# iris-ua/iris_lama

Measured on AMD Instinct MI355X. Metric: particle-scans/sec, higher is better.
Workload: dtype f64; 1 GPU; PFSlam2D 30 particles, 1080-beam synthetic corridor log (SURVEY.md 8(d)), res 0.05 m, patch 32, l2_max 0.5, GN+Cauchy(0.15), seed 42; particles=30, beams=1080, parallelism=particle-shard x1

## Files before the change

iris_lama_amd/csrc/lama_hip.hip:

```cpp
#include "../../include/lama_hip.h"

#include <hip/hip_runtime.h>

#include <algorithm>
#include <cmath>
#include <cstdio>
#include <cstdlib>
#include <cstring>
#include <map>
#include <memory>
#include <mutex>
#include <string>
#include <vector>

#include "lama_kernels.h"
#include "lama_pgo.h"
#include "lama_map_build.h"
#include "../host/pgo_pattern.hpp"

using namespace lama_dev;

namespace {

template <class T>
// ... 676 lines not shown
        size_t free_b = 0, total_b = 0;
        if (hipMemGetInfo(&free_b, &total_b) == hipSuccess && 2 * P * nWW * 2 + (1ull << 28) > free_b)
            return fail(c, LAMA_HIP_E_WINDOW, "not enough device memory to re-tile the window directories (" + std::to_string(2 * P * nWW * 2 >> 20) + " MB for a " + std::to_string(newW) + "-patch window)");
    }
    DevBuf<int16_t> nd[2];
    for (int k = 0; k < 2; ++k) {
        hipError_t e = nd[k].alloc(P * nWW);
        if (e == hipSuccess && newW != c->W) e = hipMemsetAsync(nd[k], 0xFF, P * nWW * 2, c->stream);
        if (e != hipSuccess) return hip_fail(c, e, "window directories");
    }
    const dim3 grid((unsigned)P, (unsigned)((std::max(WW, nWW) + 255) / 256));
    int16_t* const to_dm = nd[0]; int16_t* const to_occ = nd[1];
    hipLaunchKernelGGL(k_shift_window, grid, dim3(256), 0, c->stream, c->ms.dm_dir, to_dm, c->W, newW, dx, dy, WW, nWW, c->d_err);
    hipLaunchKernelGGL(k_shift_window, grid, dim3(256), 0, c->stream, c->ms.occ_dir, to_occ, c->W, newW, dx, dy, WW, nWW, c->d_err);
    {
        hipError_t e = hipGetLastError();
        if (e == hipSuccess) e = hipStreamSynchronize(c->stream);
        if (e != hipSuccess) return hip_fail(c, e, "k_shift_window");
    }
    c->ms.dm_dir.swap(nd[0]); c->ms.occ_dir.swap(nd[1]);
    if (newW != c->W) {
        c->W = newW; c->WC = newW * 32; c->cfg.window_patches = newW;
        c->ctr.window_growths += 1;
    }
    c->wx0 = (uint32_t)(nox * 32); c->wy0 = (uint32_t)(noy * 32);
    c->ctr.window_shifts += 1;
    c->ctr.window_patches = c->W;
    return LAMA_HIP_OK;
}

int32_t ensure_window(lama_hip_ctx* c, int64_t x0, int64_t x1, int64_t y0, int64_t y1)
{
    if (!c->mb_valid) { c->mbx0 = x0; c->mbx1 = x1; c->mby0 = y0; c->mby1 = y1; c->mb_valid = true; }
    else { c->mbx0 = std::min(c->mbx0, x0); c->mbx1 = std::max(c->mbx1, x1); c->mby0 = std::min(c->mby0, y0); c->mby1 = std::max(c->mby1, y1); }
    const int64_t ox = c->wx0 >> 5, oy = c->wy0 >> 5, W = c->W;
    if (c->debug_window) std::fprintf(stderr, "ensure_window: box x [%ld, %ld] y [%ld, %ld] mapped x [%ld, %ld] y [%ld, %ld] window x [%ld, %ld) y [%ld, %ld)\n", (long)x0, (long)x1, (long)y0, (long)y1, (long)c->mbx0, (long)c->mbx1, (long)c->mby0, (long)c->mby1, (long)ox, (long)(ox + W), (long)oy, (long)(oy + W));
    if (c->mbx0 >= ox && c->mbx1 < ox + W && c->mby0 >= oy && c->mby1 < oy + W) return LAMA_HIP_OK;
    const int64_t span = std::max(c->mbx1 - c->mbx0 + 1, c->mby1 - c->mby0 + 1);
    int64_t newW = W;
    if (span > W) newW = std::min<int64_t>(LAMA_HIP_MAX_WINDOW, std::max<int64_t>((span + 8 + 7) / 8 * 8, (W + W / 2 + 7) / 8 * 8));
    int64_t hx0 = c->mbx0, hx1 = c->mbx1, hy0 = c->mby0, hy1 = c->mby1;
    if (span > newW) { hx0 = x0; hx1 = x1; hy0 = y0; hy1 = y1; if (x1 - x0 + 1 > newW || y1 - y0 + 1 > newW) return LAMA_HIP_OK; }
    auto place = [&](int64_t o, int64_t lo, int64_t hi) {
        const int64_t a = hi - newW + 1, b = lo;
        int64_t no = std::min(std::max(o, a), b);
        if (no > o) no = std::min(no + 4, b); else if (no < o) no = std::max(no - 4, a);
        return no;
    };
    const int64_t nox = c->initialised ? place(ox, hx0, hx1) : (hx0 + hx1 + 1) / 2 - newW / 2;
    const int64_t noy = c->initialised ? place(oy, hy0, hy1) : (hy0 + hy1 + 1) / 2 - newW / 2;
    return regrid_window(c, (uint32_t)newW, nox, noy);
}

int32_t start_without_first_scan(lama_hip_ctx* c)
{
    if (c->initialised) return LAMA_HIP_OK;
    for (uint32_t p = 0; p < c->P; ++p) { c->h_poses[4 * p] = 1.0; c->h_poses[4 * p + 1] = 0.0; c->h_poses[4 * p + 2] = 0.0; c->h_poses[4 * p + 3] = 0.0; }
    HIPCHK(c, hipMemcpyAsync(c->d_poses, c->h_poses.data(), sizeof(double) * 4 * c->P, hipMemcpyHostToDevice, c->stream));
    c->initialised = true;
    return LAMA_HIP_OK;
}

int32_t fit_window(lama_hip_ctx* c, const Affine& mtf, uint32_t first, uint32_t count)
{
    double far = c->scan_reach;
    if (c->cfg.ray_rule == 0 && c->cfg.truncated_range > 0.0) far = std::min(far, c->cfg.truncated_range);
    const uint32_t guard_r = ((uint32_t)std::ceil(std::sqrt((double)c->max_sqdist)) + 1u + 31u) / 32u;
    const double reach = far + std::sqrt(mtf.t[0] * mtf.t[0] + mtf.t[1] * mtf.t[1]) + (double)(guard_r + 1u) * 32.0 * c->cfg.resolution;
    double xlo = 1e300, xhi = -1e300, ylo = 1e300, yhi = -1e300;
    for (uint32_t p = first; p < first + count; ++p) {
        const double x = c->h_poses[4 * p + 2], y = c->h_poses[4 * p + 3];
        xlo = std::min(xlo, x - reach); xhi = std::max(xhi, x + reach);
        ylo = std::min(ylo, y - reach); yhi = std::max(yhi, y + reach);
    }
    auto patch = [&](double w) { return (int64_t)std::floor((c->scale * w + c->off) / 32.0); };
    return ensure_window(c, patch(xlo), patch(xhi), patch(ylo), patch(yhi));
}

static unsigned xcd_grid(const lama_hip_ctx* c, uint32_t first, uint32_t count)
{
    return (first == 0 && count == c->P) ? (count + 7u) / 8u * 8u : count;
}

int32_t launch_allocation_phase(lama_hip_ctx* c, const DevParams& prm, uint32_t n, uint32_t first, uint32_t count, int alloc_only)
{
    const size_t need = (size_t)c->P * n;
    if (need > c->d_rrec.n) {
        c->d_rrec.reset(); c->d_rbbox.reset(); c->d_rchunk.reset();
        hipError_t e = c->d_rrec.alloc(need);
        if (e == hipSuccess) e = c->d_rbbox.alloc(need);
        if (e == hipSuccess) e = c->d_rchunk.alloc((size_t)c->P * ((n + 63) / 64));
        if (e != hipSuccess) { c->d_rrec.reset(); return hip_fail(c, e, "ray buffers"); }
    }
    hipLaunchKernelGGL(k_ray_hits, dim3(xcd_grid(c, first, count), (n + 255) / 256), dim3(256), 0, c->stream, prm, c->d_pts, (int)n, c->d_tfs, (int)first,
                       c->d_rrec, c->d_rbbox, alloc_only, c->d_rchunk);
    const int rw_seg = count <= 64 ? 4 : 1;
    hipLaunchKernelGGL(k_ray_alloc_walk, dim3(xcd_grid(c, first, count), (n * rw_seg + 255) / 256), dim3(256), 0, c->stream, prm, (const lama_dev::RayRec*)c->d_rrec, (int)n, (int)first, rw_seg);
    double far = c->scan_reach;
    if (c->cfg.truncated_range > 0.0) far = std::min(far, c->cfg.truncated_range);
    const int reach_cells = (int)std::ceil(far * c->scale) + 2;
    hipLaunchKernelGGL(k_occ_reverse_dir, dim3(count), dim3(256), 0, c->stream, prm, (int)first, (const double*)c->d_tfs, reach_cells,
                       c->unguarded_retry ? 1 : 0);
    return LAMA_HIP_OK;
}

static uint32_t route_places(const lama_hip_ctx* c, uint32_t count)
{
    const uint32_t slots = c->num_cus * 12u;
    if (c->route_forced || count >= slots) return c->route_cap;
    return std::min<uint32_t>(c->route_cap, std::max<uint32_t>(8u, (slots - count) / 7u));
}

int32_t run_update_maps(lama_hip_ctx* c, uint32_t n, const Affine& mtf, uint32_t first, uint32_t count)
{
    {
        const int32_t rcw = fit_window(c, mtf, first, count);
        if (rcw) return rcw;
    }
    c->last_mtf = mtf; c->last_first = first; c->last_count = count;
    if (c->recover_depth == 0) { c->saved_visit_bound = c->visit_bound; c->saved_ctr = c->ctr; }
    PinVec<double>& tfs = c->h_tfs;
    tfs.resize((size_t)c->P * 12);
    for (uint32_t p = 0; p < c->P; ++p) host_scan_tf(&c->h_poses[4 * p], mtf, &tfs[12 * (size_t)p]);
    HIPCHK(c, hipMemcpyAsync(c->d_tfs, tfs.data(), sizeof(double) * tfs.size(), hipMemcpyHostToDevice, c->stream));
    DevParams prm = make_params(c);
    bool early_lane = false;
    {
        Timer t(c, &c->ctr.ms_raycast, &c->ctr.launches_raycast);
        (void)hipMemsetAsync(c->d_slow_n, 0, 32 + sizeof(uint64_t) * 4 * c->P, c->stream);
        bool sequential = c->cfg.sequential_raycast == 1 || c->cfg.occupancy_policy == 1 ||
                          c->cfg.ray_rule == 1;
        if (!sequential && (n > 4096u || (uint64_t)n + 4096u > c->cfg.active_capacity)) sequential = true;
        if (!sequential && (uint64_t)c->visit_bound + n >= 65536u) {
            uint32_t m = 0;
            if (c->initialised) {
                (void)hipMemsetAsync(c->d_scalar, 0, sizeof(uint32_t), c->stream);
                hipLaunchKernelGGL(k_occ_max_visited, dim3(c->P), dim3(256), 0, c->stream, prm, c->d_scalar);
                HIPCHK(c, hipMemcpyAsync(&m, c->d_scalar, sizeof(uint32_t), hipMemcpyDeviceToHost, c->stream));
                HIPCHK(c, hipStreamSynchronize(c->stream));
            }
            c->visit_bound = m;
            if ((uint64_t)m + n >= 65536u) { sequential = true; c->ctr.wrap_guard_scans += 1; }
        }
        c->visit_bound = (uint32_t)std::min<uint64_t>((uint64_t)c->visit_bound + n, 65535u);
        if (sequential) c->ctr.sequential_raycast_scans += 1; else c->ctr.parallel_raycast_scans += 1;
        c->last_guarded = c->cfg.ray_rule == 0;
        if (!c->last_guarded) {
            const double side = 32.0 * c->cfg.resolution;
            const double rp = c->scan_reach / side + 2.5;
            const uint32_t bound = (uint32_t)std::min(32767.0, std::ceil(3.1416 * rp * rp));
            std::vector<CapRequest> reqs;
            for (uint32_t p = first; p < first + count; ++p) {
                const HostPart& pr = c->h_part[p];
                const uint32_t nd = std::min<uint32_t>(MAX_PATCHES, round_up32((uint32_t)c->h_counts[2 * p] + bound)), no = std::min<uint32_t>(MAX_PATCHES, round_up32((uint32_t)c->h_counts[2 * p + 1] + bound));
                if (nd > pr.dm_cap || no > pr.occ_cap) reqs.push_back(CapRequest{p, std::max(nd, pr.dm_cap), std::max(no, pr.occ_cap)});
            }
            if (!reqs.empty()) {
                const int32_t rg = set_capacities(c, reqs);
                if (rg) return rg;
                prm = make_params(c);
            }
        }
        if (sequential) {
            if (c->last_guarded) { const int32_t ra = launch_allocation_phase(c, prm, n, first, count, 1); if (ra) return ra; }
            hipLaunchKernelGGL(k_raycast, dim3(count), dim3(UM_BLOCK), 0, c->stream, prm, c->d_pts, (int)n, c->d_tfs, (int)first);
        } else {
            const bool two_waves_e = c->cfg.brushfire_waves == 2 || (c->cfg.brushfire_waves == 0 && count <= BF_TW_MAX_PARTICLES);
            early_lane = c->early_on && two_waves_e && c->cfg.brushfire_mode == 0 && first == 0 && count == c->P &&
                         count >= std::max<uint32_t>(c->route_min_count, c->early_min_count) && c->route_cap > 0;
            uint32_t host_n = 0;
            if (early_lane && c->ll_valid) {
                const uint32_t places = route_places(c, count);
                double mean = 0; for (uint32_t p = 0; p < c->P; ++p) mean += c->h_ll[p]; mean /= c->P;
                const double lim = 2.5 * std::min(mean, 0.0) - 5.0;
                std::vector<std::pair<double, uint32_t>> cand;
                for (uint32_t p = 0; p < c->P; ++p) if (c->h_ll[p] < lim) cand.emplace_back(c->h_ll[p], p);
                if (cand.size() > places) { std::partial_sort(cand.begin(), cand.begin() + places, cand.end()); cand.resize(places); }
                c->h_hlist.resize(256);
                for (auto& e : cand) c->h_hlist[host_n++] = e.second;
                if (host_n) HIPCHK(c, hipMemcpyAsync(c->d_hlist, c->h_hlist.data(), sizeof(uint32_t) * host_n, hipMemcpyHostToDevice, c->stream));
            }
            const bool prev_ok = c->early_ok && c->early_candidates > 0;
            early_lane = early_lane && (host_n > 0 || prev_ok);
            if (early_lane)
                hipLaunchKernelGGL(k_early_list, dim3(1), dim3(256), 0, c->stream, prev_ok ? (const uint8_t*)c->d_heavy : (const uint8_t*)nullptr,
                                   (const uint32_t*)c->d_hlist, host_n, c->d_early, c->d_elist, c->d_slow_n + 4, (int)c->P, route_places(c, count));
            { const int32_t ra = launch_allocation_phase(c, prm, n, first, count, 0); if (ra) return ra; }
#ifdef LAMA_WAVE_SIM
            const unsigned gy = 4u;
#else
            const unsigned gy = count <= 64 ? 128u : (count >= 1024 ? 8u : 32u);
#endif
            if (early_lane) {
                DevParams pe = prm;
                pe.elist = c->d_elist; pe.elist_n = c->d_slow_n + 4; pe.lane = 1;
                const unsigned eg = route_places(c, count);
                hipLaunchKernelGGL(k_ray_patches, dim3(eg, 128u), dim3(256), 0, c->stream, pe, (const lama_dev::RayRec*)c->d_rrec,
                                   (const uint64_t*)c->d_rbbox, (const lama_dev::RayChunk*)c->d_rchunk, (int)n, 0);
                hipLaunchKernelGGL((k_ray_replay<RP_SORT_SMALL, RP_SORT_SMALL, false, RP_BLOCK_LARGE>), dim3(eg), dim3(RP_BLOCK_LARGE), 0, c->stream, pe, 0);
                hipLaunchKernelGGL((k_ray_replay<8192, 8192, true, RP_BLOCK_LARGE>), dim3(eg), dim3(RP_BLOCK_LARGE), 0, c->stream, pe, 0);
                HIPCHK(c, hipEventRecord(c->ev_alloc, c->stream));
                HIPCHK(c, hipStreamWaitEvent(c->stream3, c->ev_alloc, 0));
                hipLaunchKernelGGL(k_mark_early, dim3(1), dim3(64), 0, c->stream3, pe);
                HIPCHK(c, hipEventRecord(c->ev_go, c->stream3));
                hipLaunchKernelGGL((k_brushfire<LQ_BIG, RQ_BIG, true, true>), dim3(eg), dim3(2 * UM_BLOCK), c->big_stage_pad, c->stream3, pe, 0, 2);
                HIPCHK(c, hipEventRecord(c->ev_early, c->stream3));
                HIPCHK(c, hipStreamWaitEvent(c->stream, c->ev_go, 0));
                prm.early = c->d_early;
            }
            hipLaunchKernelGGL(k_ray_patches, dim3(xcd_grid(c, first, count), gy), dim3(256), 0, c->stream, prm, (const lama_dev::RayRec*)c->d_rrec,
                               (const uint64_t*)c->d_rbbox, (const lama_dev::RayChunk*)c->d_rchunk, (int)n, (int)first);
            const unsigned resume_grid = std::min<unsigned>(count, 256u);
            if (count <= 512) {
                hipLaunchKernelGGL((k_ray_replay<RP_SORT_SMALL, RP_SORT_SMALL, false, RP_BLOCK_LARGE>), dim3(count), dim3(RP_BLOCK_LARGE), 0, c->stream, prm, (int)first);
                hipLaunchKernelGGL((k_ray_replay<8192, 8192, true, RP_BLOCK_LARGE>), dim3(resume_grid), dim3(RP_BLOCK_LARGE), 0, c->stream, prm, (int)first);
            } else {
                hipLaunchKernelGGL((k_ray_replay<RP_SORT_SMALL, RP_SORT_SMALL, false, RP_BLOCK_SMALL>), dim3(count), dim3(RP_BLOCK_SMALL), 0, c->stream, prm, (int)first);
                hipLaunchKernelGGL((k_ray_replay<8192, 8192, true, RP_BLOCK_SMALL>), dim3(resume_grid), dim3(RP_BLOCK_SMALL), 0, c->stream, prm, (int)first);
            }
        }
        t.stop();
    }
    HIPCHK(c, hipGetLastError());
    {
        Timer t(c, &c->ctr.ms_brushfire, &c->ctr.launches_brushfire);
        if (c->cfg.brushfire_mode == 1)
            hipLaunchKernelGGL(k_brushfire_canon, dim3(count), dim3(CN_BLOCK), 0, c->stream, prm, (int)first);
        const bool two_waves = c->cfg.brushfire_waves == 2 || (c->cfg.brushfire_waves == 0 && count <= BF_TW_MAX_PARTICLES);
        c->ctr.brushfire_mode = c->cfg.brushfire_mode;
        c->ctr.brushfire_waves = two_waves ? 2u : 1u;
        const unsigned resume_grid = std::min<unsigned>(count, 256u);
        const bool route = two_waves && count >= c->route_min_count && c->route_cap > 0;
        if (two_waves) {
            if (route) {
                prm.heavy = c->d_heavy;
                hipLaunchKernelGGL(k_bf_route, dim3(1), dim3(256), 0, c->stream, prm, (int)first, (int)count, c->route_min_events, c->route_percent, route_places(c, count));
                HIPCHK(c, hipEventRecord(c->ev_route, c->stream));
                hipLaunchKernelGGL((k_brushfire<LQ_BIG, RQ_BIG, true, true>), dim3(route_places(c, count)), dim3(2 * UM_BLOCK), 0, c->stream, prm, (int)first, 1);
                HIPCHK(c, hipStreamWaitEvent(c->stream2, c->ev_route, 0));
                hipLaunchKernelGGL((k_brushfire<LQ_SMALL, RQ_SMALL, false, true>), dim3(count), dim3(2 * UM_BLOCK), 0, c->stream2, prm, (int)first, 0);
                HIPCHK(c, hipEventRecord(c->ev_heavy, c->stream2));
                HIPCHK(c, hipStreamWaitEvent(c->stream, c->ev_heavy, 0));
            } else {
                hipLaunchKernelGGL((k_brushfire<LQ_SMALL, RQ_SMALL, false, true>), dim3(count), dim3(2 * UM_BLOCK), 0, c->stream, prm, (int)first, 0);
            }
            hipLaunchKernelGGL((k_brushfire<LQ_BIG, RQ_BIG, true, true>), dim3(resume_grid), dim3(2 * UM_BLOCK), 0, c->stream, prm, (int)first, 0);
        } else {
            hipLaunchKernelGGL((k_brushfire<LQ_SMALL, RQ_SMALL, false, false>), dim3(count), dim3(UM_BLOCK), 0, c->stream, prm, (int)first, 0);
            hipLaunchKernelGGL((k_brushfire<LQ_BIG, RQ_BIG, true, false>), dim3(resume_grid), dim3(UM_BLOCK), 0, c->stream, prm, (int)first, 0);
        }
        if (early_lane) HIPCHK(c, hipStreamWaitEvent(c->stream, c->ev_early, 0));
        hipLaunchKernelGGL(k_brushfire_slow, dim3(count), dim3(UM_BLOCK), 0, c->stream, prm, (int)first);
        c->early_ok = route && first == 0 && count == c->P;
        t.stop();
    }
    HIPCHK(c, hipGetLastError());
    return LAMA_HIP_OK;
}


int32_t permute_particles(lama_hip_ctx* c, const int32_t* idx)
{
    const uint32_t P = c->P;
    std::vector<uint8_t> taken(P, 0);
    std::vector<HostPart> np(P);
    std::vector<int32_t> nc(2 * (size_t)P);
    std::vector<double> npose(4 * (size_t)P);
    std::vector<uint32_t> clones;
    for (uint32_t i = 0; i < P; ++i) {
        const uint32_t j = (uint32_t)idx[i];
// ... 1435 lines not shown
```

iris_lama_amd/csrc/lama_raycast_par.h:

```cpp
#pragma once
#include "lama_dev.h"

namespace lama_dev {


constexpr int RP_BLOCK_SMALL = 256, RP_BLOCK_LARGE = 1024;
#ifdef LAMA_TEST_SMALL_QUEUES
constexpr int RP_SORT_SMALL = 512;
#else
constexpr int RP_SORT_SMALL = 2048;
#endif

__device__ inline int dir_alloc_one(int16_t* dir, uint32_t pidx, int32_t* count, int cap, int errbit, int32_t* err)
{
    uint32_t* w = reinterpret_cast<uint32_t*>(dir) + (pidx >> 1);
    const int sh = (int)(pidx & 1u) * 16;
    for (uint32_t spins = 0;; ++spins) {
        const uint32_t v = __hip_atomic_load(w, __ATOMIC_RELAXED, __HIP_MEMORY_SCOPE_AGENT);
        const int s = (int)(int16_t)((v >> sh) & 0xFFFFu);
        if (s >= 0) return s;
        if (s == -3) return -1;
        if (spins > (1u << 22)) { atomicOr(err, errbit); return -1; }
        if (s == -1) {
            const uint32_t locked = (v & ~(0xFFFFu << sh)) | (0xFFFEu << sh);
// ... 28 lines not shown
        const int leader = __ffsll((long long)m) - 1;
        const uint32_t klo = (uint32_t)__builtin_amdgcn_readlane((int)(uint32_t)key, leader);
        const uint32_t khi = (uint32_t)__builtin_amdgcn_readlane((int)(uint32_t)(key >> 32), leader);
        int r = 0;
        if (lane == leader) r = dir_alloc_one(dir, pidx, count, cap, errbit, err);
        r = __builtin_amdgcn_readlane(r, leader);
        if (pending && (uint32_t)key == klo && (uint32_t)(key >> 32) == khi) { res = r; pending = false; }
    }
    return res;
}

struct BeamGeom {
    uint32_t mhx, mhy, msx, msy;
    uint32_t a0, a1, nn;
    int s0, s1;
    bool mark_hit;
    int steps;
    uint64_t magic;
};

__device__ inline BeamGeom beam_geometry(const DevParams& prm, const double* T, double px, double py, double pz)
{
    double hx = ((T[0] * px + T[1] * py) + T[2] * pz) + T[9];
    double hy = ((T[3] * px + T[4] * py) + T[5] * pz) + T[10];
    double hz = ((T[6] * px + T[7] * py) + T[8] * pz) + T[11];
    double sx = T[9], sy = T[10], sz = T[11];
    double abx = 0, aby = 0, abz = 0, ray_length = 1.0;
    BeamGeom g;
    g.mark_hit = true;
    if (prm.trunc_range > 0.0) {
        abx = hx - sx; aby = hy - sy; abz = hz - sz;
        ray_length = sqrt((abx * abx + aby * aby) + abz * abz);
        if (prm.trunc_range < ray_length) {
            hx = sx + abx / ray_length * prm.trunc_range;
            hy = sy + aby / ray_length * prm.trunc_range;
            hz = sz + abz / ray_length * prm.trunc_range;
            g.mark_hit = false;
        }
    }
    if (g.mark_hit && prm.trunc_ray > 0.0) {
        if (prm.trunc_range == 0.0) {
            abx = hx - sx; aby = hy - sy; abz = hz - sz;
            ray_length = sqrt((abx * abx + aby * aby) + abz * abz);
        }
        if (prm.trunc_ray < ray_length) {
            sx = hx - abx / ray_length * prm.trunc_ray;
            sy = hy - aby / ray_length * prm.trunc_ray;
            sz = hz - abz / ray_length * prm.trunc_ray;
        }
    }
    g.mhx = w2m(prm, hx); g.mhy = w2m(prm, hy);
    g.msx = w2m(prm, sx); g.msy = w2m(prm, sy);
    const uint32_t mhz = w2m(prm, hz), msz = w2m(prm, sz);
    const int64_t d0 = (int64_t)g.mhx - (int64_t)g.msx, d1 = (int64_t)g.mhy - (int64_t)g.msy, d2 = (int64_t)mhz - (int64_t)msz;
    const int64_t a0 = d0 < 0 ? -d0 : d0, a1 = d1 < 0 ? -d1 : d1, a2 = d2 < 0 ? -d2 : d2;
    const int64_t nn = a0 > a1 ? (a0 > a2 ? a0 : a2) : (a1 > a2 ? a1 : a2);
    g.s0 = d0 < 0 ? -1 : 1; g.s1 = d1 < 0 ? -1 : 1;
    g.a0 = (uint32_t)a0; g.a1 = (uint32_t)a1; g.nn = (uint32_t)(nn > 0xFFFFFFFFll ? 0xFFFFFFFFll : nn);
    g.steps = nn > 0 ? (int)g.nn - 1 : 0;
    if (nn >= 8192) g.steps = -1;
    g.magic = (1ull << 42) / (uint64_t)(2 * (nn > 0 && nn < 8192 ? nn : 1)) + 1ull;
    return g;
}

constexpr int ACT_SEQ_BITS = 26, ACT_XY_BITS = 15;
__device__ inline uint64_t act_key(uint32_t rx, uint32_t ry, uint32_t beam, uint32_t t)
{
    return ((uint64_t)((ry << ACT_XY_BITS) | rx) << ACT_SEQ_BITS) | (uint64_t)((beam << 13) | t);
}

__device__ inline void act_append(const DevParams& prm, int p, uint64_t key)
{
    const uint32_t k = atomicAdd(prm.act_count + p, 1u);
    if (k < prm.act_cap) prm.act[(size_t)p * prm.act_cap + k] = key;
    else atomicOr(prm.err, ERR_QUEUE);
}

struct RayRec;
struct RayChunk;
constexpr uint64_t RAY_BBOX_EMPTY = 0x0000FFFF0000FFFFull;
__device__ inline uint64_t ray_hits_record(const DevParams& prm, const BeamGeom& g, int p, int i, int n, RayRec* rec_out, uint64_t* bbox_out);
__device__ inline void ray_chunk_record(const DevParams& prm, const BeamGeom& g, uint64_t bb, int lane, RayChunk* chunks, size_t index);

__global__ __launch_bounds__(256) void k_ray_hits(DevParams prm, const double* __restrict__ pts, int n,
                                                   const double* __restrict__ tfs, int first_particle,
                                                   RayRec* __restrict__ rec_out = nullptr, uint64_t* __restrict__ bbox_out = nullptr, int alloc_only = 0,
                                                   RayChunk* __restrict__ chunk_out = nullptr)
{
    const int p = first_particle + blockIdx.x;
    if (p >= (int)prm.P) return;
    const int i = blockIdx.y * 256 + threadIdx.x;
    const int lane = threadIdx.x & 63;
    const bool live = i < n;
    const int ic = live ? i : n - 1;
    double T[12];
    uload_f64_w<12>(tfs + 12 * (size_t)p, T);
    const BeamGeom g = beam_geometry(prm, T, pts[3 * ic], pts[3 * ic + 1], pts[3 * ic + 2]);
    uint64_t bb = RAY_BBOX_EMPTY;
    if (rec_out && live) bb = ray_hits_record(prm, g, p, i, n, rec_out, bbox_out);
    if (chunk_out && (i & ~63) < n) ray_chunk_record(prm, g, bb, lane, chunk_out, (size_t)p * ((n + 63) / 64) + (i >> 6));
    if (live && g.steps < 0) atomicOr(prm.err, ERR_WINDOW);
    if (!alloc_only) {
        uint32_t st = (live && g.steps > 0) ? (uint32_t)g.steps : 0u;
        for (int off = 32; off > 0; off >>= 1) st += (uint32_t)__shfl_xor((int)st, off, 64);
        if (lane == 0 && st) atomicAdd((unsigned long long*)(prm.stats + 4 * p + 2), (unsigned long long)st);
    }
    bool hit = live && g.steps >= 0 && g.mark_hit;
    const uint32_t rx = g.mhx - prm.wx0, ry = g.mhy - prm.wy0;
    if (hit && (rx >= prm.WC || ry >= prm.WC)) { atomicOr(prm.err, ERR_WINDOW); hit = false; }
    const uint32_t pidx = (ry >> 5) * prm.W + (rx >> 5), ci = (rx & 31u) | ((ry & 31u) << 5);
    int slot = -1;
    const PV pv = pview(prm, p);
    if (hit) slot = dir_get_or_alloc(pv.occ_dir, pidx, prm.counts + 2 * p + 1, (int)pv.occ_cap, ERR_OCC_CAP, prm.err);
    hit = hit && slot >= 0 && !alloc_only;
    if (hit) atomicOr((unsigned long long*)(pv.occ_hit + (size_t)slot * 16 + (ci >> 6)), 1ull << (ci & 63));
    const unsigned long long hm = __ballot(hit);
    if (hm) {
        uint32_t base = 0;
        if (lane == (__ffsll((long long)hm) - 1)) base = atomicAdd(prm.act_count + p, (uint32_t)__popcll(hm));
        base = (uint32_t)__shfl((int)base, __ffsll((long long)hm) - 1, 64);
        if (hit) {
            const uint32_t k = base + (uint32_t)__popcll(hm & ((1ull << lane) - 1ull));
            if (k < prm.act_cap) prm.act[(size_t)p * prm.act_cap + k] = act_key(rx, ry, (uint32_t)i, 0u);
            else atomicOr(prm.err, ERR_QUEUE);
        }
    }
}

template <int RP_BLOCK>
__device__ inline void bitonic_sort(uint64_t* a, uint32_t m)
{
    for (uint32_t k = 2; k <= m; k <<= 1) {
        for (uint32_t j = k >> 1; j > 0; j >>= 1) {
            for (uint32_t i = threadIdx.x; i < m; i += RP_BLOCK) {
                const uint32_t ixj = i ^ j;
                if (ixj > i) {
                    const uint64_t x = a[i], y = a[ixj];
                    const bool up = (i & k) == 0;
                    if ((x > y) == up) { a[i] = y; a[ixj] = x; }
                }
            }
            __syncthreads();
        }
    }
}

template <int RP_BLOCK, int E>
__device__ inline void bitonic_sort_regs(uint64_t* a)
{
    constexpr uint32_t M = (uint32_t)RP_BLOCK * E;
    const uint32_t base = threadIdx.x * (uint32_t)E;
    uint64_t x[E];
#pragma unroll
    for (int r = 0; r < E; ++r) x[r] = a[base + r];
    for (uint32_t k = 2; k <= M; k <<= 1) {
        uint32_t j = k >> 1;
        for (; j >= 64u * E; j >>= 1) {
            __syncthreads();
#pragma unroll
            for (int r = 0; r < E; ++r) a[base + r] = x[r];
            __syncthreads();
            const uint32_t pb = base ^ j;
            const bool keep_min = ((base & j) == 0) == ((base & k) == 0);
#pragma unroll
            for (int r = 0; r < E; ++r) {
                const uint64_t y = a[pb + r];
                x[r] = ((y < x[r]) == keep_min) ? y : x[r];
            }
        }
        for (; j >= (uint32_t)E; j >>= 1) {
            const int lj = (int)(j / (uint32_t)E);
            const bool keep_min = ((base & j) == 0) == ((base & k) == 0);
#pragma unroll
            for (int r = 0; r < E; ++r) {
                const uint64_t y = __shfl_xor(x[r], lj, 64);
                x[r] = ((y < x[r]) == keep_min) ? y : x[r];
            }
        }
#pragma unroll
        for (int jr = E / 2; jr > 0; jr >>= 1) {
            if ((uint32_t)jr >= k) continue;
#pragma unroll
            for (int r = 0; r < E; ++r) {
                if (r & jr) continue;
                const bool up = ((base + (uint32_t)r) & k) == 0;
                const uint64_t lo = x[r], hi = x[r | jr];
                const bool sw = (lo > hi) == up;
                x[r] = sw ? hi : lo; x[r | jr] = sw ? lo : hi;
            }
        }
    }
    __syncthreads();
#pragma unroll
    for (int r = 0; r < E; ++r) a[base + r] = x[r];
    __syncthreads();
}

template <int RP_BLOCK>
__device__ inline void sort_keys(uint64_t* a, uint32_t m)
{
    if (m < (uint32_t)RP_BLOCK) { if (m > 1) bitonic_sort<RP_BLOCK>(a, m); }
    else if (m == (uint32_t)RP_BLOCK) bitonic_sort_regs<RP_BLOCK, 1>(a);
    else if (m == 2u * RP_BLOCK) bitonic_sort_regs<RP_BLOCK, 2>(a);
    else if (m == 4u * RP_BLOCK) bitonic_sort_regs<RP_BLOCK, 4>(a);
    else if (m == 8u * RP_BLOCK) bitonic_sort_regs<RP_BLOCK, 8>(a);
    else bitonic_sort<RP_BLOCK>(a, m);
}

template <int SORT_CAP, int EV_CAP>
// ... 150 lines not shown
```

iris_lama_amd/csrc/lama_raycast_patch.h:

```cpp
#pragma once
#include "lama_raycast_par.h"

namespace lama_dev {

struct RayRec {
    uint32_t msx, msy;
    uint32_t a01;
    uint32_t nnf;
    uint64_t magic;
};
struct RayChunk {
    int32_t cwx, cwy;
    int32_t ccwx, ccwy;
    uint64_t bbox;
    uint32_t sxy;
    uint32_t cone;
};

__device__ inline RayRec ray_rec(const BeamGeom& g)
{
    RayRec r;
    r.msx = g.msx; r.msy = g.msy;
    r.a01 = (g.a0 & 0xFFFFu) | ((g.a1 & 0xFFFFu) << 16);
    r.nnf = (g.nn & 0xFFFFu) | (g.s0 < 0 ? 1u << 16 : 0u) | (g.s1 < 0 ? 1u << 17 : 0u) | (g.steps > 0 ? 1u << 18 : 0u);
    r.magic = g.magic;
    return r;
}
__device__ __forceinline__ void ray_cell(const RayRec& r, uint32_t wx0, uint32_t wy0, uint32_t t, uint32_t& rx, uint32_t& ry)
{
    const uint32_t a0 = r.a01 & 0xFFFFu, a1 = r.a01 >> 16, nn = r.nnf & 0xFFFFu;
    const uint32_t st0 = (uint32_t)(((uint64_t)(2u * t * a0 + nn) * r.magic) >> 42);
    const uint32_t st1 = (uint32_t)(((uint64_t)(2u * t * a1 + nn) * r.magic) >> 42);
    const uint32_t cx = (r.nnf & (1u << 16)) ? r.msx - st0 : r.msx + st0;
    const uint32_t cy = (r.nnf & (1u << 17)) ? r.msy - st1 : r.msy + st1;
    rx = cx - wx0; ry = cy - wy0;
}

__device__ __forceinline__ bool ray_axis_range(int m, bool neg, uint32_t a, uint32_t nn, int lo, uint32_t steps, uint32_t& t_lo, uint32_t& t_hi)
{
    int ka = neg ? m - (lo + 31) : lo - m, kb = neg ? m - lo : lo + 31 - m;
    if (ka < 0) ka = 0;
    if (kb > (int)a) kb = (int)a;
    if (ka > kb) return false;
    t_lo = 1u; t_hi = steps;
    if (a == 0u) return true;
    const uint32_t d = 2u * a;
    if (ka > 0) t_lo = (2u * nn * (uint32_t)ka - nn + d - 1u) / d;
    if (kb < (int)a) t_hi = (2u * nn * (uint32_t)(kb + 1) - nn + d - 1u) / d - 1u;
    if (t_lo < 1u) t_lo = 1u;
    if (t_hi > steps) t_hi = steps;
    return t_lo <= t_hi;
}

__device__ inline uint64_t ray_hits_record(const DevParams& prm, const BeamGeom& g, int p, int i, int n, RayRec* rec_out, uint64_t* bbox_out)
{
    RayRec r = ray_rec(g);
    uint64_t bb = RAY_BBOX_EMPTY;
    bool ok = g.steps > 0;
    if (ok) {
        const int64_t xa = (int64_t)g.msx - (int64_t)prm.wx0, ya = (int64_t)g.msy - (int64_t)prm.wy0;
        const int64_t xb = xa + (int64_t)g.s0 * (int64_t)g.a0, yb = ya + (int64_t)g.s1 * (int64_t)g.a1;
        const int64_t x0 = xa < xb ? xa : xb, x1 = xa < xb ? xb : xa, y0 = ya < yb ? ya : yb, y1 = ya < yb ? yb : ya;
        if (x0 < 0 || y0 < 0 || x1 >= (int64_t)prm.WC || y1 >= (int64_t)prm.WC) { atomicOr(prm.err, ERR_WINDOW); ok = false; }
        else bb = (uint64_t)x0 | ((uint64_t)x1 << 16) | ((uint64_t)y0 << 32) | ((uint64_t)y1 << 48);
    }
    if (!ok) r.nnf &= ~(1u << 18);
    rec_out[(size_t)p * n + i] = r;
    bbox_out[(size_t)p * n + i] = bb;
    return bb;
}

__device__ inline void ray_chunk_record(const DevParams& prm, const BeamGeom& g, uint64_t bb, int lane, RayChunk* chunks, size_t index)
{
    const bool val = bb != RAY_BBOX_EMPTY;
    const unsigned long long vm = __ballot(val);
    uint32_t x0 = (uint32_t)(bb & 0xFFFFu), x1 = (uint32_t)((bb >> 16) & 0xFFFFu), y0 = (uint32_t)((bb >> 32) & 0xFFFFu), y1 = (uint32_t)(bb >> 48);
    for (int off = 32; off > 0; off >>= 1) {
        const uint32_t ox0 = (uint32_t)__shfl_xor((int)x0, off, 64), ox1 = (uint32_t)__shfl_xor((int)x1, off, 64);
        const uint32_t oy0 = (uint32_t)__shfl_xor((int)y0, off, 64), oy1 = (uint32_t)__shfl_xor((int)y1, off, 64);
        x0 = ox0 < x0 ? ox0 : x0; x1 = ox1 > x1 ? ox1 : x1; y0 = oy0 < y0 ? oy0 : y0; y1 = oy1 > y1 ? oy1 : y1;
    }
    const int lf = vm ? __ffsll((long long)vm) - 1 : 0, ll = vm ? 63 - __clzll((long long)vm) : 0;
    const int dx = g.s0 < 0 ? -(int)g.a0 : (int)g.a0, dy = g.s1 < 0 ? -(int)g.a1 : (int)g.a1;
    const int sx = (int)(g.msx - prm.wx0), sy = (int)(g.msy - prm.wy0);
    const int fx = __shfl(dx, lf, 64), fy = __shfl(dy, lf, 64), lx = __shfl(dx, ll, 64), ly = __shfl(dy, ll, 64);
    const int fsx = __shfl(sx, lf, 64), fsy = __shfl(sy, lf, 64);
    const int c_f = fx * dy - fy * dx, c_l = dx * ly - dy * lx;
    const bool front = fx * dx + fy * dy > 0 && lx * dx + ly * dy > 0 && sx == fsx && sy == fsy;
    const bool all_ccw = __ballot(val && !(front && c_f >= 0 && c_l >= 0)) == 0ull;
    const bool all_cw = __ballot(val && !(front && c_f <= 0 && c_l <= 0)) == 0ull;
    if (lane == 0) {
        RayChunk c;
        c.bbox = vm ? ((uint64_t)x0 | ((uint64_t)x1 << 16) | ((uint64_t)y0 << 32) | ((uint64_t)y1 << 48)) : RAY_BBOX_EMPTY;
        c.sxy = ((uint32_t)fsx & 0xFFFFu) | ((uint32_t)fsy << 16);
        c.cone = (vm && (all_ccw || all_cw)) ? 1u : 0u;
        c.cwx = all_ccw ? fx : lx; c.cwy = all_ccw ? fy : ly;
        c.ccwx = all_ccw ? lx : fx; c.ccwy = all_ccw ? ly : fy;
        chunks[index] = c;
    }
}

__global__ __launch_bounds__(256) void k_ray_alloc_walk(DevParams prm, const RayRec* __restrict__ recs, int n, int first_particle, int RW_SEG)
{
    const int p = first_particle + blockIdx.x;
    const int g = blockIdx.y * 256 + threadIdx.x;
    const int i = g / RW_SEG, seg = g % RW_SEG;
    if (i >= n || p >= (int)prm.P) return;
    const RayRec r = recs[(size_t)p * n + i];
    if (!(r.nnf & (1u << 18))) return;
    const uint32_t steps = (r.nnf & 0xFFFFu) - 1u;
    const uint32_t t0 = 1u + (uint32_t)(((uint64_t)steps * (uint32_t)seg) / RW_SEG), t1 = (uint32_t)(((uint64_t)steps * (uint32_t)(seg + 1)) / RW_SEG);
    const PV pv = pview(prm, p);
    int16_t* occ_dir = pv.occ_dir;
    if (t0 > t1) return;
    const uint32_t a0 = r.a01 & 0xFFFFu, a1 = r.a01 >> 16, nn = r.nnf & 0xFFFFu;
    const uint32_t k0 = (uint32_t)(((uint64_t)(2u * t0 * a0 + nn) * r.magic) >> 42), k1 = (uint32_t)(((uint64_t)(2u * t0 * a1 + nn) * r.magic) >> 42);
    const bool neg0 = (r.nnf >> 16) & 1u, neg1 = (r.nnf >> 17) & 1u;
    const uint32_t bx = r.msx - prm.wx0, by = r.msy - prm.wy0;
    const uint32_t rx = neg0 ? bx - k0 : bx + k0, ry = neg1 ? by - k1 : by + k1;
    uint32_t X = rx >> 5, Y = ry >> 5;
    uint32_t kx = neg0 ? k0 + (rx & 31u) + 1u : k0 + 32u - (rx & 31u), ky = neg1 ? k1 + (ry & 31u) + 1u : k1 + 32u - (ry & 31u);
    auto step_of = [nn](uint32_t k, uint32_t a) { return k > a ? 0xFFFFFFFFu : (2u * nn * k - nn + 2u * a - 1u) / (2u * a); };
    uint32_t tx = step_of(kx, a0), ty = step_of(ky, a1);
    (void)dir_get_or_alloc(occ_dir, Y * prm.W + X, prm.counts + 2 * p + 1, (int)pv.occ_cap, ERR_OCC_CAP, prm.err);
    for (;;) {
        const uint32_t t = tx < ty ? tx : ty;
        if (t > t1) break;
        if (tx == t) { X = neg0 ? X - 1u : X + 1u; kx += 32u; tx = step_of(kx, a0); }
        if (ty == t) { Y = neg1 ? Y - 1u : Y + 1u; ky += 32u; ty = step_of(ky, a1); }
        (void)dir_get_or_alloc(occ_dir, Y * prm.W + X, prm.counts + 2 * p + 1, (int)pv.occ_cap, ERR_OCC_CAP, prm.err);
    }
}

__device__ inline int imin(int a, int b) { return a < b ? a : b; }
__device__ inline int imax(int a, int b) { return a > b ? a : b; }
constexpr int RD_MARK_SIDE = 256;
constexpr int RD_MARK_WORDS = RD_MARK_SIDE * RD_MARK_SIDE / 32;

__global__ __launch_bounds__(256) void k_occ_reverse_dir(DevParams prm, int first_particle,
                                                          const double* __restrict__ tfs , int reach_cells, int guard_off)
{
    __shared__ uint32_t mark[RD_MARK_WORDS];
    __shared__ uint32_t need_s;
    const int p = first_particle + blockIdx.x;
    const uint32_t W = prm.W, WW = W * W;
    const int tid = threadIdx.x, r = (int)prm.guard_r;
    const PV pv = pview_w(prm, p);
    const int16_t* occ_dir = pv.occ_dir;
    const int16_t* dm_dir = pv.dm_dir;
    const int scx = (int)(w2m(prm, uload_f64(tfs + 12 * (size_t)p + 9)) - prm.wx0), scy = (int)(w2m(prm, uload_f64(tfs + 12 * (size_t)p + 10)) - prm.wy0);
    const int bx0 = imax((scx - reach_cells) >> 5, 0), bx1 = imin((scx + reach_cells) >> 5, (int)W - 1);
    const int by0 = imax((scy - reach_cells) >> 5, 0), by1 = imin((scy + reach_cells) >> 5, (int)W - 1);
    const int mx0 = imax(bx0 - r, 0), my0 = imax(by0 - r, 0), mw = imin(bx1 + r, (int)W - 1) - mx0 + 1, mh = imin(by1 + r, (int)W - 1) - my0 + 1;
    const bool bounded = mw > 0 && mh > 0 && mw <= RD_MARK_SIDE && mh <= RD_MARK_SIDE;
    const uint32_t nbits = bounded ? (uint32_t)(mw * mh) : 0u;
    for (uint32_t i = tid; i < (nbits + 31u) / 32u; i += 256u) mark[i] = 0;
    if (tid == 0) need_s = 0;
    __syncthreads();
    for (uint32_t w0 = (uint32_t)tid * 8u; w0 < WW; w0 += 256u * 8u) {
        const uint4 q = *reinterpret_cast<const uint4*>(occ_dir + w0);
        if ((q.x & q.y & q.z & q.w) == 0xFFFFFFFFu) continue;
        const uint32_t ww[4] = {q.x, q.y, q.z, q.w};
        const int wy = (int)(w0 / W), x0 = (int)(w0 % W);
#pragma unroll
        for (int k = 0; k < 8; ++k) {
            const int slot = (int)(int16_t)((ww[k >> 1] >> ((k & 1) * 16)) & 0xFFFFu);
            if (slot < 0) continue;
            pv.rev[slot] = (int32_t)(w0 + (uint32_t)k);
            if (!bounded || x0 + k < bx0 || x0 + k > bx1 || wy < by0 || wy > by1) continue;
            for (int dy = -r; dy <= r; ++dy)
                for (int dx = -r; dx <= r; ++dx) {
                    const int x = x0 + k + dx - mx0, y = wy + dy - my0;
                    if ((uint32_t)x < (uint32_t)mw && (uint32_t)y < (uint32_t)mh) { const uint32_t n = (uint32_t)y * (uint32_t)mw + (uint32_t)x; atomicOr(&mark[n >> 5], 1u << (n & 31u)); }
                }
        }
    }
    __syncthreads();
    uint32_t need = 0;
    for (uint32_t i = tid; i < (nbits + 31u) / 32u; i += 256u) {
        uint32_t m = mark[i];
        while (m) {
            const uint32_t n = i * 32u + (uint32_t)(__ffs((int)m) - 1);
            const uint32_t wx = (uint32_t)mx0 + n % (uint32_t)mw, wy = (uint32_t)my0 + n / (uint32_t)mw;
            if (dm_dir[wy * W + wx] < 0) ++need;
            m &= m - 1u;
        }
    }
    if (need) atomicAdd(&need_s, need);
    __syncthreads();
    if (tid == 0) prm.guard[p] = bounded ? need_s : 0u;
    if (tid == 0 && bounded && !guard_off && (uint64_t)prm.counts[2 * p] + need_s > pv.dm_cap) atomicOr(prm.err, ERR_DM_CAP);
}

#ifdef LAMA_PROFILE_RAY
#ifdef LAMA_PROFILE_RAY_COUNT
#define RPC(k, v) atomicAdd((unsigned long long*)(prm.dbg + 16 * (size_t)prm.P + (k)), (unsigned long long)(v))
#else
#define RPC(k, v) do {} while (0)
#endif
#define RPT_T(k) do { if (tid == 0) { const uint64_t t_ = __builtin_readcyclecounter(); tacc[(k) - 8] += t_ - tprev; tprev = t_; } } while (0)
#else
#define RPC(k, v) do {} while (0)
#define RPT_T(k) do {} while (0)
#endif
constexpr int RPT_CHUNK = 256;
#ifndef LAMA_RPT_WALK
#define LAMA_RPT_WALK 4
#endif
constexpr int RPT_WALK = LAMA_RPT_WALK;

__global__ __launch_bounds__(256, 6) void k_ray_patches(DevParams prm, const RayRec* __restrict__ recs, const uint64_t* __restrict__ bbox,
                                                      const RayChunk* __restrict__ chunks, int n, int first_particle)
{
    static_assert(RPT_CHUNK == 256, "one candidate beam per thread and round");
    __shared__ uint32_t cnt[1024];
    __shared__ RayRec lrec[RPT_CHUNK];
    __shared__ uint32_t lbt[RPT_CHUNK];
    __shared__ uint16_t lbeam[RPT_CHUNK];
    __shared__ uint32_t actw[32], newm[32], wrapm[32];
    __shared__ uint32_t list_n[2];
    const int p = lane_particle(prm, first_particle, (int)blockIdx.x);
    const int tid = threadIdx.x, lane = tid & 63, wave = tid >> 6;
    if (map_update_aborted(prm)) { if (blockIdx.x == 0 && blockIdx.y == 0 && tid == 0) atomicOr(prm.err, ERR_CLEAN_ABORT); return; }
    if (p < 0) return;
    const int count = prm.counts[2 * p + 1];
    const PVOcc pv = pview_occ_w(prm, p);
    uint32_t* occ = pv.occ;
    const RayRec* prec = recs + (size_t)p * n;
    const uint64_t* pbb = bbox + (size_t)p * n;
    const int nck = (n + 63) / 64;
    RayChunk ck;
    ck.bbox = RAY_BBOX_EMPTY; ck.cone = 0; ck.cwx = ck.cwy = ck.ccwx = ck.ccwy = 0; ck.sxy = 0;
    if (lane < nck) ck = chunks[(size_t)p * nck + lane];
    if (tid < 2) list_n[tid] = 0;
    int slot = blockIdx.y;
    uint32_t pidx_next = slot < count ? (uint32_t)pv.rev[slot] : 0u;
    uint32_t par = 0;
#ifdef LAMA_PROFILE_RAY
    uint64_t tacc[8] = {0, 0, 0, 0, 0, 0, 0, 0}, tprev = 0;
#endif
    __syncthreads();
    for (; slot < count; slot += gridDim.y) {
        const uint32_t pidx = pidx_next;
        if (slot + (int)gridDim.y < count) pidx_next = (uint32_t)pv.rev[slot + gridDim.y];
        const int px = (int)((pidx % prm.W) * 32u), py = (int)((pidx / prm.W) * 32u);
#ifdef LAMA_PROFILE_RAY
        tprev = __builtin_readcyclecounter();
        ++tacc[5];
        if (tid == 0) RPC(0, 1);
#endif
        bool keep = false;
        if (lane < nck) {
            const int x0 = (int)(ck.bbox & 0xFFFFu), x1 = (int)((ck.bbox >> 16) & 0xFFFFu), y0 = (int)((ck.bbox >> 32) & 0xFFFFu), y1 = (int)(ck.bbox >> 48);
            keep = !(x1 < px || x0 > px + 31 || y1 < py || y0 > py + 31);
            if (keep && ck.cone) {
                const int sx = (int)(ck.sxy & 0xFFFFu), sy = (int)(ck.sxy >> 16);
                const int ax = px - 1 - sx, bx = px + 32 - sx, ay = py - 1 - sy, by = py + 32 - sy;
                const int a00 = ck.cwx * ay - ck.cwy * ax, a10 = ck.cwx * ay - ck.cwy * bx, a01 = ck.cwx * by - ck.cwy * ax, a11 = ck.cwx * by - ck.cwy * bx;
                const int b00 = ck.ccwx * ay - ck.ccwy * ax, b10 = ck.ccwx * ay - ck.ccwy * bx, b01 = ck.ccwx * by - ck.ccwy * ax, b11 = ck.ccwx * by - ck.ccwy * bx;
                if ((a00 < 0 && a10 < 0 && a01 < 0 && a11 < 0) || (b00 > 0 && b10 > 0 && b01 > 0 && b11 > 0)) keep = false;
            }
        }
        const unsigned long long km = __ballot(keep);
        const int ncand = __popcll(km) * 64;
        if (tid == 0) RPC(2, __popcll(km));
        if (km == 0ull) continue;
        uint32_t v[4];
        uint64_t hw[4];
        const uint64_t* hitw = pv.occ_hit + (size_t)slot * 16;
#pragma unroll
        for (int j = 0; j < 4; ++j) { v[j] = occ[(size_t)slot * 1024 + tid + 256 * j]; hw[j] = hitw[wave + 4 * j]; }
        bool has_act = false;
        for (int c0 = 0; c0 == 0 || c0 < ncand; c0 += RPT_CHUNK, par ^= 1u) {
            const int jc = (c0 >> 6) + wave;
// ... 117 lines not shown
```

Baseline: 16880 particle-scans/s.

## Fuse ray hits, alloc walk and reverse-dir into one per-particle kernel

For small particle counts, the three allocation-phase kernels (ray hits, allocation walk, occupancy reverse directory) are merged into a single k_ray_prepare kernel with one 1024-thread block per particle. The stages are separated by block-level fences and barriers instead of kernel boundaries. The memset of the slow-path counters and stats is folded into the kernel when the whole particle set is processed. This removes launch overhead and one memset per scan, but each particle now runs on a single block, so the raycast stages get less parallelism than the previous multi-block grids.

New measurement: 16690 particle-scans/s. -1.1%, worse.

```diff
diff --git a/iris_lama_amd/csrc/lama_hip.hip b/iris_lama_amd/csrc/lama_hip.hip
--- a/iris_lama_amd/csrc/lama_hip.hip
+++ b/iris_lama_amd/csrc/lama_hip.hip
@@ -782,7 +782,8 @@
     return (first == 0 && count == c->P) ? (count + 7u) / 8u * 8u : count;
 }
 
-int32_t launch_allocation_phase(lama_hip_ctx* c, const DevParams& prm, uint32_t n, uint32_t first, uint32_t count, int alloc_only)
+static bool fused_prepare(uint32_t count, int alloc_only) { return count <= 64 && !alloc_only; }
+int32_t launch_allocation_phase(lama_hip_ctx* c, const DevParams& prm, uint32_t n, uint32_t first, uint32_t count, int alloc_only, uint32_t zero_mask = 0)
 {
     const size_t need = (size_t)c->P * n;
     if (need > c->d_rrec.n) {
@@ -792,13 +793,19 @@
         if (e == hipSuccess) e = c->d_rchunk.alloc((size_t)c->P * ((n + 63) / 64));
         if (e != hipSuccess) { c->d_rrec.reset(); return hip_fail(c, e, "ray buffers"); }
     }
-    hipLaunchKernelGGL(k_ray_hits, dim3(xcd_grid(c, first, count), (n + 255) / 256), dim3(256), 0, c->stream, prm, c->d_pts, (int)n, c->d_tfs, (int)first,
-                       c->d_rrec, c->d_rbbox, alloc_only, c->d_rchunk);
     const int rw_seg = count <= 64 ? 4 : 1;
-    hipLaunchKernelGGL(k_ray_alloc_walk, dim3(xcd_grid(c, first, count), (n * rw_seg + 255) / 256), dim3(256), 0, c->stream, prm, (const lama_dev::RayRec*)c->d_rrec, (int)n, (int)first, rw_seg);
     double far = c->scan_reach;
     if (c->cfg.truncated_range > 0.0) far = std::min(far, c->cfg.truncated_range);
     const int reach_cells = (int)std::ceil(far * c->scale) + 2;
+    if (fused_prepare(count, alloc_only)) {
+        hipLaunchKernelGGL(k_ray_prepare, dim3(count), dim3(RPREP_BLOCK), 0, c->stream, prm, c->d_pts, (int)n, c->d_tfs, (int)first,
+                           (lama_dev::RayRec*)c->d_rrec, (uint64_t*)c->d_rbbox, (lama_dev::RayChunk*)c->d_rchunk, rw_seg, reach_cells,
+                           c->unguarded_retry ? 1 : 0, zero_mask);
+        return LAMA_HIP_OK;
+    }
+    hipLaunchKernelGGL(k_ray_hits, dim3(xcd_grid(c, first, count), (n + 255) / 256), dim3(256), 0, c->stream, prm, c->d_pts, (int)n, c->d_tfs, (int)first,
+                       c->d_rrec, c->d_rbbox, alloc_only, c->d_rchunk);
+    hipLaunchKernelGGL(k_ray_alloc_walk, dim3(xcd_grid(c, first, count), (n * rw_seg + 255) / 256), dim3(256), 0, c->stream, prm, (const lama_dev::RayRec*)c->d_rrec, (int)n, (int)first, rw_seg);
     hipLaunchKernelGGL(k_occ_reverse_dir, dim3(count), dim3(256), 0, c->stream, prm, (int)first, (const double*)c->d_tfs, reach_cells,
                        c->unguarded_retry ? 1 : 0);
     return LAMA_HIP_OK;
@@ -827,7 +834,6 @@
     bool early_lane = false;
     {
         Timer t(c, &c->ctr.ms_raycast, &c->ctr.launches_raycast);
-        (void)hipMemsetAsync(c->d_slow_n, 0, 32 + sizeof(uint64_t) * 4 * c->P, c->stream);
         bool sequential = c->cfg.sequential_raycast == 1 || c->cfg.occupancy_policy == 1 ||
                           c->cfg.ray_rule == 1;
         if (!sequential && (n > 4096u || (uint64_t)n + 4096u > c->cfg.active_capacity)) sequential = true;
@@ -844,6 +850,8 @@
         }
         c->visit_bound = (uint32_t)std::min<uint64_t>((uint64_t)c->visit_bound + n, 65535u);
         if (sequential) c->ctr.sequential_raycast_scans += 1; else c->ctr.parallel_raycast_scans += 1;
+        const bool zero_in_kernel = !sequential && fused_prepare(count, 0) && first == 0 && count == c->P;
+        if (!zero_in_kernel) (void)hipMemsetAsync(c->d_slow_n, 0, 32 + sizeof(uint64_t) * 4 * c->P, c->stream);
         c->last_guarded = c->cfg.ray_rule == 0;
         if (!c->last_guarded) {
             const double side = 32.0 * c->cfg.resolution;
@@ -885,7 +893,7 @@
             if (early_lane)
                 hipLaunchKernelGGL(k_early_list, dim3(1), dim3(256), 0, c->stream, prev_ok ? (const uint8_t*)c->d_heavy : (const uint8_t*)nullptr,
                                    (const uint32_t*)c->d_hlist, host_n, c->d_early, c->d_elist, c->d_slow_n + 4, (int)c->P, route_places(c, count));
-            { const int32_t ra = launch_allocation_phase(c, prm, n, first, count, 0); if (ra) return ra; }
+            { const int32_t ra = launch_allocation_phase(c, prm, n, first, count, 0, zero_in_kernel ? (early_lane ? 0xEFu : 0xFFu) : 0u); if (ra) return ra; }
 #ifdef LAMA_WAVE_SIM
             const unsigned gy = 4u;
 #else
diff --git a/iris_lama_amd/csrc/lama_raycast_par.h b/iris_lama_amd/csrc/lama_raycast_par.h
--- a/iris_lama_amd/csrc/lama_raycast_par.h
+++ b/iris_lama_amd/csrc/lama_raycast_par.h
@@ -134,19 +134,12 @@
 __device__ inline uint64_t ray_hits_record(const DevParams& prm, const BeamGeom& g, int p, int i, int n, RayRec* rec_out, uint64_t* bbox_out);
 __device__ inline void ray_chunk_record(const DevParams& prm, const BeamGeom& g, uint64_t bb, int lane, RayChunk* chunks, size_t index);
 
-__global__ __launch_bounds__(256) void k_ray_hits(DevParams prm, const double* __restrict__ pts, int n,
-                                                   const double* __restrict__ tfs, int first_particle,
-                                                   RayRec* __restrict__ rec_out = nullptr, uint64_t* __restrict__ bbox_out = nullptr, int alloc_only = 0,
-                                                   RayChunk* __restrict__ chunk_out = nullptr)
-{
-    const int p = first_particle + blockIdx.x;
-    if (p >= (int)prm.P) return;
-    const int i = blockIdx.y * 256 + threadIdx.x;
+__device__ inline void ray_hits_beam(const DevParams& prm, const double* __restrict__ pts, int n, const double (&T)[12], int p, int i,
+                                     RayRec* rec_out, uint64_t* bbox_out, int alloc_only, RayChunk* chunk_out)
+{
     const int lane = threadIdx.x & 63;
     const bool live = i < n;
     const int ic = live ? i : n - 1;
-    double T[12];
-    uload_f64_w<12>(tfs + 12 * (size_t)p, T);
     const BeamGeom g = beam_geometry(prm, T, pts[3 * ic], pts[3 * ic + 1], pts[3 * ic + 2]);
     uint64_t bb = RAY_BBOX_EMPTY;
     if (rec_out && live) bb = ray_hits_record(prm, g, p, i, n, rec_out, bbox_out);
@@ -177,6 +170,18 @@
             else atomicOr(prm.err, ERR_QUEUE);
         }
     }
+}
+
+__global__ __launch_bounds__(256) void k_ray_hits(DevParams prm, const double* __restrict__ pts, int n,
+                                                   const double* __restrict__ tfs, int first_particle,
+                                                   RayRec* __restrict__ rec_out = nullptr, uint64_t* __restrict__ bbox_out = nullptr, int alloc_only = 0,
+                                                   RayChunk* __restrict__ chunk_out = nullptr)
+{
+    const int p = first_particle + blockIdx.x;
+    if (p >= (int)prm.P) return;
+    double T[12];
+    uload_f64_w<12>(tfs + 12 * (size_t)p, T);
+    ray_hits_beam(prm, pts, n, T, p, blockIdx.y * 256 + threadIdx.x, rec_out, bbox_out, alloc_only, chunk_out);
 }
 
 template <int RP_BLOCK>
diff --git a/iris_lama_amd/csrc/lama_raycast_patch.h b/iris_lama_amd/csrc/lama_raycast_patch.h
--- a/iris_lama_amd/csrc/lama_raycast_patch.h
+++ b/iris_lama_amd/csrc/lama_raycast_patch.h
@@ -100,10 +100,8 @@
     }
 }
 
-__global__ __launch_bounds__(256) void k_ray_alloc_walk(DevParams prm, const RayRec* __restrict__ recs, int n, int first_particle, int RW_SEG)
-{
-    const int p = first_particle + blockIdx.x;
-    const int g = blockIdx.y * 256 + threadIdx.x;
+__device__ inline void ray_alloc_walk_stretch(const DevParams& prm, const RayRec* recs, int n, int p, int g, int RW_SEG)
+{
     const int i = g / RW_SEG, seg = g % RW_SEG;
     if (i >= n || p >= (int)prm.P) return;
     const RayRec r = recs[(size_t)p * n + i];
@@ -131,33 +129,36 @@
         (void)dir_get_or_alloc(occ_dir, Y * prm.W + X, prm.counts + 2 * p + 1, (int)pv.occ_cap, ERR_OCC_CAP, prm.err);
     }
 }
+__global__ __launch_bounds__(256) void k_ray_alloc_walk(DevParams prm, const RayRec* __restrict__ recs, int n, int first_particle, int RW_SEG)
+{
+    ray_alloc_walk_stretch(prm, recs, n, first_particle + (int)blockIdx.x, (int)(blockIdx.y * 256 + threadIdx.x), RW_SEG);
+}
 
 __device__ inline int imin(int a, int b) { return a < b ? a : b; }
 __device__ inline int imax(int a, int b) { return a > b ? a : b; }
 constexpr int RD_MARK_SIDE = 256;
 constexpr int RD_MARK_WORDS = RD_MARK_SIDE * RD_MARK_SIDE / 32;
 
-__global__ __launch_bounds__(256) void k_occ_reverse_dir(DevParams prm, int first_particle,
-                                                          const double* __restrict__ tfs , int reach_cells, int guard_off)
-{
-    __shared__ uint32_t mark[RD_MARK_WORDS];
-    __shared__ uint32_t need_s;
-    const int p = first_particle + blockIdx.x;
+template <int NT>
+__device__ inline void occ_reverse_dir_particle(const DevParams& prm, int p, double sx, double sy, int reach_cells, int guard_off,
+                                                uint32_t* mark ,
+                                                uint32_t& need_s)
+{
     const uint32_t W = prm.W, WW = W * W;
     const int tid = threadIdx.x, r = (int)prm.guard_r;
     const PV pv = pview_w(prm, p);
     const int16_t* occ_dir = pv.occ_dir;
     const int16_t* dm_dir = pv.dm_dir;
-    const int scx = (int)(w2m(prm, uload_f64(tfs + 12 * (size_t)p + 9)) - prm.wx0), scy = (int)(w2m(prm, uload_f64(tfs + 12 * (size_t)p + 10)) - prm.wy0);
+    const int scx = (int)(w2m(prm, sx) - prm.wx0), scy = (int)(w2m(prm, sy) - prm.wy0);
     const int bx0 = imax((scx - reach_cells) >> 5, 0), bx1 = imin((scx + reach_cells) >> 5, (int)W - 1);
     const int by0 = imax((scy - reach_cells) >> 5, 0), by1 = imin((scy + reach_cells) >> 5, (int)W - 1);
     const int mx0 = imax(bx0 - r, 0), my0 = imax(by0 - r, 0), mw = imin(bx1 + r, (int)W - 1) - mx0 + 1, mh = imin(by1 + r, (int)W - 1) - my0 + 1;
     const bool bounded = mw > 0 && mh > 0 && mw <= RD_MARK_SIDE && mh <= RD_MARK_SIDE;
     const uint32_t nbits = bounded ? (uint32_t)(mw * mh) : 0u;
-    for (uint32_t i = tid; i < (nbits + 31u) / 32u; i += 256u) mark[i] = 0;
+    for (uint32_t i = tid; i < (nbits + 31u) / 32u; i += (uint32_t)NT) mark[i] = 0;
     if (tid == 0) need_s = 0;
     __syncthreads();
-    for (uint32_t w0 = (uint32_t)tid * 8u; w0 < WW; w0 += 256u * 8u) {
+    for (uint32_t w0 = (uint32_t)tid * 8u; w0 < WW; w0 += (uint32_t)NT * 8u) {
         const uint4 q = *reinterpret_cast<const uint4*>(occ_dir + w0);
         if ((q.x & q.y & q.z & q.w) == 0xFFFFFFFFu) continue;
         const uint32_t ww[4] = {q.x, q.y, q.z, q.w};
@@ -177,7 +178,7 @@
     }
     __syncthreads();
     uint32_t need = 0;
-    for (uint32_t i = tid; i < (nbits + 31u) / 32u; i += 256u) {
+    for (uint32_t i = tid; i < (nbits + 31u) / 32u; i += (uint32_t)NT) {
         uint32_t m = mark[i];
         while (m) {
             const uint32_t n = i * 32u + (uint32_t)(__ffs((int)m) - 1);
@@ -190,6 +191,43 @@
     __syncthreads();
     if (tid == 0) prm.guard[p] = bounded ? need_s : 0u;
     if (tid == 0 && bounded && !guard_off && (uint64_t)prm.counts[2 * p] + need_s > pv.dm_cap) atomicOr(prm.err, ERR_DM_CAP);
+}
+__global__ __launch_bounds__(256) void k_occ_reverse_dir(DevParams prm, int first_particle,
+                                                          const double* __restrict__ tfs , int reach_cells, int guard_off)
+{
+    __shared__ uint32_t mark[RD_MARK_WORDS];
+    __shared__ uint32_t need_s;
+    const int p = first_particle + blockIdx.x;
+    occ_reverse_dir_particle<256>(prm, p, uload_f64(tfs + 12 * (size_t)p + 9), uload_f64(tfs + 12 * (size_t)p + 10), reach_cells, guard_off, mark, need_s);
+}
+
+constexpr int RPREP_BLOCK = 1024;
+__global__ __launch_bounds__(RPREP_BLOCK) void k_ray_prepare(DevParams prm, const double* __restrict__ pts, int n, const double* __restrict__ tfs,
+                                                             int first_particle, RayRec* rrec, uint64_t* rbbox, RayChunk* rchunk, int RW_SEG,
+                                                             int reach_cells, int guard_off, uint32_t zero_mask)
+{
+    __shared__ uint32_t mark[RD_MARK_WORDS];
+    __shared__ uint32_t need_s;
+    const int p = first_particle + blockIdx.x;
+    const int tid = threadIdx.x;
+    double T[12];
+    uload_f64_w<12>(tfs + 12 * (size_t)p, T);
+    if (zero_mask) {
+        if (blockIdx.x == 0 && tid < 8 && ((zero_mask >> tid) & 1u)) prm.slow_n[tid] = 0;
+        if (tid < 4) prm.stats[4 * p + tid] = 0;
+        __threadfence();
+        __syncthreads();
+    }
+    for (int base = 0; base < n; base += RPREP_BLOCK) {
+        const int i = base + tid;
+        if ((i & ~63) < n) ray_hits_beam(prm, pts, n, T, p, i, rrec, rbbox, 0, rchunk);
+    }
+    __threadfence();
+    __syncthreads();
+    for (int g = tid; g < n * RW_SEG; g += RPREP_BLOCK) ray_alloc_walk_stretch(prm, rrec, n, p, g, RW_SEG);
+    __threadfence();
+    __syncthreads();
+    occ_reverse_dir_particle<RPREP_BLOCK>(prm, p, T[9], T[10], reach_cells, guard_off, mark, need_s);
 }
 
 #ifdef LAMA_PROFILE_RAY
```
